# Mourtz/raytracer-0

Measured on AMD Instinct MI355X. Metric: Msamples/sec (pixels x spp / s) at 1024^2 Cornell, 8 bounces, higher is better.
Workload: dtype f32; 1 GPU; c2 (c2_cornell_mis_8): BASELINE configs[1] (the headline): 1024x1024 Cornell, MIS power heuristic, MAX_BOUNCES = MAX_DIFF_BOUNCES = 8, 64 spp; width=1024, height=1024, spp=64, max_diff_bounces=8, parallelism=row-band x1 (16-row bands), kernel=scene-specialised (hipRTC JIT), executor_compat=False

## Files before the change

raytracer-0_amd/csrc/rt0_integrator.h:

```cpp
#pragma once
#ifndef RT0_JIT
#include <hip/hip_runtime.h>
#include "rt0_device.h"
#endif

#define DEV __device__ __forceinline__

namespace rt0 {

constexpr float EPSILON = 0.001f;
constexpr float INF_T = 1e4f;
constexpr float F_INF = __builtin_huge_valf();
constexpr float PI_F = 3.14159265f;
constexpr float ONE_OVER_PI = 0.31830989f;
constexpr float TWO_PI = 6.28318531f;
constexpr float FOUR_PI = 12.5663706f;
constexpr float VOL_SIGMA_T = 0.15f;
constexpr float VOL_SIGMA_S = 0.13f;
constexpr float VOL_G = 0.5f;

enum { T_SPHERE = 0, T_PLANE = 1, T_BOX = 2, T_SDF = 3, T_TRIANGLE = 5 };
enum { M_LIGHT = 0, M_DIR_LIGHT = 1, M_DIFF = 2, M_SPEC = 3, M_REFR_FRESNEL = 4, M_REFR_SCHLICK = 5, M_COAT = 6 };

struct v3 {
  float x, y, z;
};
DEV v3 mk(float x, float y, float z) { return v3{x, y, z}; }
DEV v3 operator+(v3 a, v3 b) { return mk(a.x + b.x, a.y + b.y, a.z + b.z); }
DEV v3 operator-(v3 a, v3 b) { return mk(a.x - b.x, a.y - b.y, a.z - b.z); }
DEV v3 operator*(v3 a, v3 b) { return mk(a.x * b.x, a.y * b.y, a.z * b.z); }
DEV v3 operator*(v3 a, float s) { return mk(a.x * s, a.y * s, a.z * s); }
DEV float dot(v3 a, v3 b) { return a.x * b.x + a.y * b.y + a.z * b.z; }
DEV float frcp(float x) { return __builtin_amdgcn_rcpf(x); }
DEV float frsq(float x) { return __builtin_amdgcn_rsqf(x); }
DEV float fsqrt(float x) { return __builtin_amdgcn_sqrtf(x); }
DEV float fdiv(float a, float b) { return a * frcp(b); }
DEV float sgn(float x) { return x > 0.0f ? 1.0f : (x < 0.0f ? -1.0f : 0.0f); }
DEV float step_(float e, float x) { return x < e ? 0.0f : 1.0f; }
DEV float mixf(float x, float y, float a) { return a * (y - x) + x; }
DEV v3 normalize(v3 a) { return a * frsq(dot(a, a)); }
DEV float length(v3 a) { return fsqrt(dot(a, a)); }
DEV v3 vmaxs(v3 a, float s) { return mk(fmaxf(a.x, s), fmaxf(a.y, s), fmaxf(a.z, s)); }
DEV float vmaxc(v3 a) { return fmaxf(a.x, fmaxf(a.y, a.z)); }
DEV v3 vabs(v3 a) { return mk(fabsf(a.x), fabsf(a.y), fabsf(a.z)); }
DEV v3 reflect(v3 i, v3 n) { return i - n * (2.0f * dot(n, i)); }
DEV v3 refract(v3 i, v3 n, float eta) {
  float d = dot(n, i);
  float k = 1.0f - eta * eta * (1.0f - d * d);
  if (k < 0.0f) return mk(0.f, 0.f, 0.f);
  return i * eta - n * (eta * d + fsqrt(k));
}
DEV float fsin(float x) { return __sinf(x); }
DEV float fcos(float x) { return __cosf(x); }
DEV float fsin_rev(float t) { return __builtin_amdgcn_sinf(t); }
DEV float fcos_rev(float t) { return __builtin_amdgcn_cosf(t); }
DEV float fexp(float x) { return __expf(x); }
DEV float flog(float x) { return __logf(x); }

#ifndef RT0_HALO_CHECK
#define RT0_HALO_CHECK 1
#endif
#ifndef RT0_DEFER_NEE
#define RT0_DEFER_NEE 0
#endif
#ifndef RT0_NEE_REGIONS
#define RT0_NEE_REGIONS 2
#endif
#ifndef RT0_TAP_BATCH
#define RT0_TAP_BATCH 1
#endif
#ifndef RT0_NEE_WALK
#define RT0_NEE_WALK 0
#endif
#ifndef RT0_WALK_ROOT_TEST
#define RT0_WALK_ROOT_TEST 1
#endif
#define RT0_RES_STRIDE 2
#ifndef RT0_TREELET
#define RT0_TREELET 0
#endif
#ifndef RT0_BVH_STACK16
#define RT0_BVH_STACK16 0
#endif
#ifndef RT0_WAVEFRONT
#define RT0_WAVEFRONT 0
#endif
#ifndef RT0_WF_REFILL
#define RT0_WF_REFILL 1
#endif
#ifndef RT0_WF_WALK_REFILL
#define RT0_WF_WALK_REFILL 16
#endif
#ifndef RT0_WF_INLINE_NODES
#define RT0_WF_INLINE_NODES 1
#endif
#ifndef RT0_WF_UNIT
#define RT0_WF_UNIT 256
#endif
DEV float nc_fract(float x) {
#pragma clang fp contract(off)
  return x - floorf(x);
}
DEV float nc_addmul(float a, float b, float c) {
#pragma clang fp contract(off)
  return a + (b * c);
}
DEV float nc_seed4(float s, float a, float f, float b, float c, float d) {
#pragma clang fp contract(off)
  return ((s + (a * f)) + b) + (c * d);
}
DEV float nc_seed3(float s, float a, float f, float c, float d) {
#pragma clang fp contract(off)
  return (s + (a * f)) + (c * d);
}

DEV float hash(float seed) {
#pragma clang fp contract(off)
  uint32_t n = __float_as_uint(seed) * 747796405u + 2891336453u;
  n = ((n >> ((n >> 28u) + 4u)) ^ n) * 277803737u;
  const uint32_t m = (n >> 22u) ^ n;
  const float lo = (float)(int32_t)(m & 0x7fffffffu);
  const float hi = __int_as_float((int32_t)m >> 31 & 0x3f000000);
  return __builtin_fmaf(lo, 2.3283064365386963e-10f, hi);
}
DEV void hash2(float sx, float sy, float &ox, float &oy) {
#pragma clang fp contract(off)
  float x = (sx * 0.1031f), y = (sy * 0.1030f);
  x = x - floorf(x);
  y = y - floorf(y);
  float d = (x * (y + 19.19f)) + (y * (x + 19.19f));
  x += d;
  y += d;
  float a = ((x + y) * x), b = ((x + y) * y);
  ox = a - floorf(a);
  oy = b - floorf(b);
}

struct DynScene {
  static constexpr bool kStatic = false;
  static constexpr int kMeshes = 0, kSdfs = 0, kLights = 0;
  static constexpr bool kMayHaveModels = true;
  const SceneDev *__restrict__ S;
  DEV int n_meshes() const { return S->n_meshes; }
  DEV int n_sdfs() const { return S->n_sdfs; }
  DEV int n_models() const { return S->n_models; }
  DEV int n_lights() const { return S->n_lights; }
  DEV GeomRec geom(int i) const { return S->geom[i]; }
  DEV MatRec mat(int i) const { return S->mat[i]; }
  DEV float j3(int i) const { return S->j3[i]; }
  DEV int sdf_kind(int i) const { return S->sdf_kind[i]; }
  DEV int light(int i) const { return S->light_index[i]; }
  DEV bool any_tex() const { return S->any_tex != 0; }
  DEV TexRec tex(int i) const { return S->tex[i]; }
};

struct DynCfg {
  uint32_t fl;
  int mb, md, ms, mt, msc, mst, rs;
  float fud;
  DEV explicit DynCfg(const LaunchParams &P)
      : fl(P.flags), mb(P.max_bounces), md(P.max_diff), ms(P.max_spec), mt(P.max_trans), msc(P.max_scatter),
        mst(P.marching_steps), rs(P.restir_samples), fud(P.fudge) {}
  DEV uint32_t flags() const { return fl; }
  DEV int max_bounces() const { return mb; }
  DEV int max_diff() const { return md; }
  DEV int max_spec() const { return ms; }
  DEV int max_trans() const { return mt; }
  DEV int max_scatter() const { return msc; }
  DEV int marching_steps() const { return mst; }
  DEV int restir_samples() const { return rs; }
  DEV float fudge() const { return fud; }
};

template <int I, int N, class F>
DEV void static_for(F &&f) {
  if constexpr (I < N) {
    f(I);
    static_for<I + 1, N>(f);
  }
}
template <class Scene, class F>
DEV void for_meshes(const Scene &sc, F &&f) {
  if constexpr (Scene::kStatic) static_for<0, Scene::kMeshes>(f);
  else
    for (int i = 0; i < sc.n_meshes(); ++i) f(i);
}
template <class Scene, class F>
DEV void for_lights(const Scene &sc, F &&f) {
  if constexpr (Scene::kStatic) static_for<0, Scene::kLights>(f);
  else
    for (int i = 0; i < sc.n_lights(); ++i) f(i);
}
template <class Scene, class F>
DEV void for_sdfs(const Scene &sc, F &&f) {
  if constexpr (Scene::kStatic) static_for<0, Scene::kSdfs>(f);
  else
    for (int i = 0; i < sc.n_sdfs(); ++i) f(i);
}

struct Hit {
  v3 n, pos;
  int index;
  int type;
};

#ifndef RT0_MARCH_BUDGET
#define RT0_MARCH_BUDGET 12
#endif

struct March {
  v3 o, d;
  float tmin, t, id;
  int i;
  bool active, done;
  v3 n;
};

DEV v3 ray_at(v3 o, v3 d, float t) {
  return v3{__builtin_fmaf(d.x, t, o.x), __builtin_fmaf(d.y, t, o.y), __builtin_fmaf(d.z, t, o.z)};
}

DEV float sdBox(v3 p, v3 b) {
  v3 d = vabs(p) - b;
  v3 m = mk(fmaxf(d.x, 0.f), fmaxf(d.y, 0.f), fmaxf(d.z, 0.f));
  return length(m) + fminf(fmaxf(d.x, fmaxf(d.y, d.z)), 0.0f);
}
DEV float sdCone(v3 p, v3 c) {
  float qx = fsqrt(p.x * p.x + p.z * p.z), qy = p.y;
  float d1 = -qy - c.z;
  float d2 = fmaxf(qx * c.x + qy * c.y, qy);
  float a = fmaxf(d1, 0.f), b = fmaxf(d2, 0.f);
  return fsqrt(a * a + b * b) + fminf(fmaxf(d1, d2), 0.f);
}
DEV float gmod(float x, float y) { return x - y * floorf(x * frcp(y)); }
DEV float menger(v3 p, v3 scale) {
  float d = sdBox(p, scale);
  float s = 1.0f;
#pragma unroll
  for (int m = 0; m < 4; ++m) {
    v3 ps = p * s;
    v3 a = mk(gmod(ps.x, 2.0f) - 1.0f, gmod(ps.y, 2.0f) - 1.0f, gmod(ps.z, 2.0f) - 1.0f);
    s *= 3.0f;
    v3 r = mk(fabsf(1.0f - 3.0f * fabsf(a.x)), fabsf(1.0f - 3.0f * fabsf(a.y)), fabsf(1.0f - 3.0f * fabsf(a.z)));
    float da = fmaxf(r.x, r.y), db = fmaxf(r.y, r.z), dc = fmaxf(r.z, r.x);
    float c = (fminf(da, fminf(db, dc)) - 1.0f) / s;
    d = fmaxf(c, d);
  }
  return d;
}
DEV float mandelbulb(v3 p) {
// ... 1648 lines not shown
      spec = true;
    } else if (mt.type == M_COAT) {
      float nt_eff = fabsf(mt.nt);
      if constexpr (SPECTRAL) {
        if (flag(F_SPECTRAL) && mt.nt < 0.0f) nt_eff = spectral_ior(hero, fabsf(mt.nt));
      }
      spec = hash(seed) < schlick(gr_rd, gr_nl, 1.00029f, nt_eff);
    }
    if (spec || !flag(F_SAMPLE_LIGHTS) || !flag(F_RESTIR_DEF)) return;
    if (flag(F_RESTIR) && flag(F_MIS)) {
      if (sc.n_lights() <= 8) return;
    } else if (!flag(F_RESTIR)) {
      return;
    }
    const float fr = (float)frame;
    restir<true>(gr_x, gr_nl, mt, nc_seed3(seed, 8652.1f, fr, gr_bounce, 7895.13f),
                 nc_seed3(seed, 1234.567f, fr, gr_bounce, 9876.54f));
  }
  DEV bool ghost_on() const { return RESTIR && (C.flags() & F_EXEC_GHOST) != 0; }

  DEV bool quad_rec() const { return !RESTIR && (C.flags() & F_EXEC_GHOST) != 0 && P.quad_mode != 0; }
  DEV int light_q(int i, float bounce) {
    const int li = sc.light(i);
    if (!quad_rec()) return li;
    const int d = (int)bounce;
    if (d >= 32) return li;
    if (i == 0) q_own |= 1u << d;
    if (!q0_on || sc.n_lights() < 2) return li;
    const uint32_t m = q0_m | (flag(F_VOL) ? 0u : q0_g);
    if ((m >> d) & 1u) return li;
    if (flag(F_VOL) && (m & ((1u << d) - 1u)) == 0u) return sc.light(0);
    return 0;
  }
  DEV void quad_ghost(float seed, int depth) {
    if (!gr_have || depth >= 32) return;
    const MatRec mt = sc.mat(gr_mat);
    bool spec = gr_spec;
    if (mt.type == M_DIFF) {
      spec = false;
    } else if (mt.type == M_SPEC || mt.type == M_REFR_FRESNEL || mt.type == M_REFR_SCHLICK) {
      spec = true;
    } else if (mt.type == M_COAT) {
      float nt_eff = fabsf(mt.nt);
      if constexpr (SPECTRAL) {
        if (flag(F_SPECTRAL) && mt.nt < 0.0f) nt_eff = spectral_ior(hero, fabsf(mt.nt));
      }
      spec = hash(seed) < schlick(gr_rd, gr_nl, 1.00029f, nt_eff);
    }
    if (!spec && flag(F_SAMPLE_LIGHTS) && !flag(F_RESTIR) && !(flag(F_MIS) && sc.n_lights() > 0) &&
        sc.n_lights() <= 4)
      q_gown |= 1u << depth;
  }
  DEV void quad_begin() {
    if (!quad_rec()) return;
    q_own = q_gown = 0u;
    gr_have = false;
    q0_on = P.quad_mode == 2 && ((q_px | q_py) & 1) != 0;
    if (q0_on) {
      const uint2 m = P.quad_masks[(size_t)(q_py & ~1) * P.width + (q_px & ~1)];
      q0_m = m.x;
      q0_g = m.y;
    }
  }
  DEV void quad_store() const {
    if (quad_rec() && P.quad_mode == 1) P.quad_masks[(size_t)q_py * P.width + q_px] = make_uint2(q_own, q_gown);
  }

  DEV void wf_emit_shadow(int l, v3 o, v3 d, float tq, v3 c, bool dirl) {
    const uint32_t i = wave_append(wf_wave_counter(1));
    float4 *e = P.wf_sh + 3 * ((size_t)wf_region * (uint32_t)P.wf_R * (uint32_t)P.wf_L + i);
    e[0] = make_float4(o.x, o.y, o.z, tq);
    e[1] = make_float4(d.x, d.y, d.z, __uint_as_float((uint32_t)l * P.wf_slots + wf_slot));
    e[2] = make_float4(c.x, c.y, c.z, dirl ? 1.0f : 0.0f);
    wf_bits |= 1u << l;
  }
  DEV void wf_nee_surface(v3 x, v3 nl, float seed, float bounce) {
    if (flag(F_RESTIR)) return;
    const float fr = (float)frame;
    const float base = nc_seed4(seed, 8652.1f, fr, 5681.123f, bounce, 7895.13f);
    wf_kind = 1;
    for_lights(sc, [&](int i) {
      const int idx = sc.light(i);
      if (idx < 0) return;
      WfShadow wj{mk(0.f, 0.f, 0.f), mk(0.f, 0.f, 0.f), -1.0f, false};
      if (flag(F_MIS)) {
        const GeomRec lg = sc.geom(idx);
        const MatRec lmt = sc.mat(idx);
        if (lmt.type != M_LIGHT) return;
        LightGeo geo{false, 0.f, 0.f, 0.f, mk(0.f, 0.f, 0.f)};
        const v3 ls = direct_light(idx, x, nl, nc_addmul(base, (float)i, 123.456f), nullptr, nullptr, &geo, false, &wj);
        if (!(dot(ls, ls) > 0.000001f) || wj.tq < 0.0f) return;
        float w;
        if (geo.sphere && !flag(F_ANIM)) {
          float lp = 0.0f;
          if (geo.d2 > geo.r2 && 1.0f - geo.cam >= 1e-6f) lp = frcp(TWO_PI * (1.0f - geo.cam));
          w = power_heuristic(lp, cos_pdf(geo.ld, nl));
        } else {
          const v3 ld = normalize(lpos(idx, lg) - x);
          w = power_heuristic(light_pdf(lg, lmt, x), cos_pdf(ld, nl));
        }
        wf_emit_shadow(i, wj.o, wj.d, wj.tq, ls * w, wj.dirl);
      } else {
        const v3 dl = direct_light(idx, x, nl, base, nullptr, nullptr, nullptr, false, &wj);
        if ((dl.x != 0.0f || dl.y != 0.0f || dl.z != 0.0f) && wj.tq >= 0.0f) wf_emit_shadow(i, wj.o, wj.d, wj.tq, dl, wj.dirl);
      }
    });
  }
  DEV void wf_nee_volume(v3 sp, v3 rd, v3 mask, float seed, int depth) {
    wf_kind = 2;
    for_lights(sc, [&](int li) {
      const int lidx = sc.light(li);
      if (lidx < 0) return;
      const GeomRec lg = sc.geom(lidx);
      const MatRec lmt = sc.mat(lidx);
      if (lmt.type != M_LIGHT || lg.type != T_SPHERE) return;
      v3 dlc = mk(lg.px, lg.py, lg.pz) - sp;
      float dc = length(dlc);
      float cam = fsqrt(1.0f - fminf(fmaxf(fdiv(lg.d0, dc * dc), 0.0f), 1.0f));
      float idc = frcp(dc);
      v3 dir = sample_cone(mk(dlc.x * idc, dlc.y * idc, dlc.z * idc), 1.0f - cam,
                           nc_addmul(nc_addmul(seed + 2341.7f, (float)li, 917.3f), (float)depth, 199.1f));
      Hit sh;
      const v3 so = sp + dir * (EPSILON * 20.0f);
      float ts = isect_q(so, dir, sh);
      if (sh.index != lidx) return;
      float omega = 2.0f * (1.0f - cam);
      float ct = dot(rd, dir);
      constexpr float g2 = VOL_G * VOL_G;
      float den = 1.0f + g2 - 2.0f * VOL_G * ct;
      float phase = fdiv(1.0f - g2, FOUR_PI * den * fsqrt(den));
      float Tf = fexp(-VOL_SIGMA_T * ts);
      const v3 c = ((((mask * mk(lmt.cr, lmt.cg, lmt.cb)) * mk(lmt.er, lmt.eg, lmt.eb)) * phase) * Tf) * (PI_F * omega);
      wf_emit_shadow(li, so, dir, ts, c, false);
    });
  }

  static constexpr bool WF = RT0_WAVEFRONT != 0 && SDF && !RESTIR && !COUNT;
  static constexpr bool SUSP = SDF && !RESTIR && !COUNT && !WF;
  static constexpr bool WFB = RT0_WAVEFRONT != 0 && RESTIR && !SDF && !COUNT && Scene::kMayHaveModels;
  struct NeeCtx {
    v3 x, n, acc;
    float seed;
    int li;
    bool vol, end;
  };
  struct Path {
    v3 ro, rd, acc, mask, prev_nl;
    float seed;
    int depth;
    bool spec;
    int phase;
    March ms;
    NeeCtx nc;
  };
  DEV March *march_slot(Path &ps) {
    if constexpr (WFB) return (sc.n_models() > 0 && P.n_tris > 0) ? &ps.ms : nullptr;
    if constexpr (!SUSP && !WF) return nullptr;
    if constexpr (Scene::kMayHaveModels)
      if (sc.n_models() > 0 && P.n_tris > 0) return nullptr;
    return &ps.ms;
  }
  DEV void march_pending(Path &ps) {
    March &m = ps.ms;
    if (!m.active) return;
    const int cap = C.marching_steps();
    float t = m.t, id = m.id;
    int i = m.i;
    const int lim = min(cap, i + RT0_MARCH_BUDGET);
    bool stop = i >= cap;
    for (; i < lim; ++i) {
      float dist = G::map(sc, ray_at(m.o, m.d, t), id, n_map);
      float h = fabsf(dist);
      if (h < EPSILON || t > m.tmin) {
        stop = true;
        break;
      }
      t = __builtin_fmaf(h, C.fudge(), t);
    }
    if (i >= cap) stop = true;
    m.t = t;
    m.id = id;
    m.i = i;
    if (stop) {
      m.active = false;
      m.done = true;
    }
  }
  DEV bool nee_phase(Path &ps) {
    NeeCtx &nc = ps.nc;
    March *mq = march_slot(ps);
    bool susp = false;
    if (VOL && nc.vol) {
      const v3 sp = nc.x, rd = nc.n;
      const float seed = ps.seed;
      const int depth = ps.depth;
      for_lights(sc, [&](int li) {
        if (susp || li < nc.li) return;
        int lidx = sc.light(li);
        if (lidx < 0) return;
        const GeomRec lg = sc.geom(lidx);
        const MatRec lmt = sc.mat(lidx);
        if (lmt.type != M_LIGHT || lg.type != T_SPHERE) return;
        v3 dlc = mk(lg.px, lg.py, lg.pz) - sp;
        float dc = length(dlc);
        float cam = fsqrt(1.0f - fminf(fmaxf(fdiv(lg.d0, dc * dc), 0.0f), 1.0f));
        float idc = frcp(dc);
        v3 dir = sample_cone(mk(dlc.x * idc, dlc.y * idc, dlc.z * idc), 1.0f - cam,
                             nc_addmul(nc_addmul(seed + 2341.7f, (float)li, 917.3f), (float)depth, 199.1f));
        Hit sh;
        float ts = isect(sp + dir * (EPSILON * 20.0f), dir, sh, mq);
        if (mq && ts < 0.0f) {
          nc.li = li;
          susp = true;
          return;
        }
        if (sh.index != lidx) return;
        float omega = 2.0f * (1.0f - cam);
        float ct = dot(rd, dir);
        constexpr float g2 = VOL_G * VOL_G;
        float den = 1.0f + g2 - 2.0f * VOL_G * ct;
        float phase = fdiv(1.0f - g2, FOUR_PI * den * fsqrt(den));
        float Tf = fexp(-VOL_SIGMA_T * ts);
        ps.acc = ps.acc + ((((ps.mask * mk(lmt.cr, lmt.cg, lmt.cb)) * mk(lmt.er, lmt.eg, lmt.eb)) * phase) * Tf) *
                              (PI_F * omega);
      });
      return !susp;
    }
    if (!flag(F_RESTIR)) {
      if (flag(F_MIS) && sc.n_lights() > 0) {
        for_lights(sc, [&](int i) {
          if (susp || i < nc.li) return;
          int idx = light_q(i, (float)ps.depth);
          if (idx < 0) return;
          const GeomRec lg = sc.geom(idx);
          const MatRec lmt = sc.mat(idx);
          if (lmt.type != M_LIGHT) return;
          v3 ls = direct_light(idx, nc.x, nc.n, nc_addmul(nc.seed, (float)i, 123.456f), mq, &susp);
          if (susp) {
            nc.li = i;
            return;
          }
          if (dot(ls, ls) > 0.000001f) {
            v3 ld = normalize(lpos(idx, lg) - nc.x);
            nc.acc = nc.acc + ls * power_heuristic(light_pdf(lg, lmt, nc.x), cos_pdf(ld, nc.n));
          }
        });
      } else {
        for_lights(sc, [&](int i) {
          if (susp || i < nc.li) return;
          int idx = light_q(i, (float)ps.depth);
          if (idx < 0) return;
          v3 dl = direct_light(idx, nc.x, nc.n, nc.seed, mq, &susp);
          if (susp) {
            nc.li = i;
            return;
          }
          nc.acc = nc.acc + dl;
        });
      }
    }
    if (susp) return false;
    ps.acc = ps.acc + nc.acc * ps.mask;
    return true;
  }
  DEV bool step(Path &ps) {
    if constexpr (SUSP) {
      if (ps.phase == 1) {
        if (!nee_phase(ps)) return true;
        ps.phase = 0;
        return ps.nc.end ? false : ++ps.depth < C.max_bounces();
      }
    }
    v3 &ro = ps.ro, &rd = ps.rd, &acc = ps.acc, &mask = ps.mask, &prev_nl = ps.prev_nl;
    bool &spec = ps.spec;
    const float seed = ps.seed;
    const int depth = ps.depth;
    const float fr = (float)frame;
    {
    if (COUNT) ++n_iter;
    Hit hit;
    float t = isect(ro, rd, hit, march_slot(ps));
    if ((SUSP || WF || WFB) && t < 0.0f) return true;
    if constexpr (VOL) {
      if (flag(F_VOL)) {
        float sd = -flog(fmaxf(hash(nc_addmul(seed + 4729.3f, (float)depth, 991.1f)), 1e-6f)) / VOL_SIGMA_T;
        if (sd < fminf(INF_T, t)) {
          v3 sp = ro + rd * sd;
          mask = mask * (VOL_SIGMA_S / VOL_SIGMA_T);
          if constexpr (WF) {
            const v3 rd_in = rd;
            rd = sample_hg(rd, nc_addmul(seed + 8293.7f, (float)depth, 773.3f));
            ro = sp;
            spec = false;
            ++scat_ev;
            const bool stop = scat_ev >= C.max_scatter() || vmaxc(mask) < 0.01f;
            if (flag(F_SAMPLE_LIGHTS)) wf_nee_volume(sp, rd_in, mask, seed, depth);
            return stop ? false : ++ps.depth < C.max_bounces();
          }
          if constexpr (SUSP) {
            const v3 rd_in = rd;
            rd = sample_hg(rd, nc_addmul(seed + 8293.7f, (float)depth, 773.3f));
            ro = sp;
            spec = false;
            ++scat_ev;
            const bool stop = scat_ev >= C.max_scatter() || vmaxc(mask) < 0.01f;
            if (flag(F_SAMPLE_LIGHTS)) {
              ps.nc = NeeCtx{sp, rd_in, mk(0.f, 0.f, 0.f), seed, 0, true, stop};
              ps.phase = 1;
              if (!nee_phase(ps)) return true;
              ps.phase = 0;
            }
            return stop ? false : ++ps.depth < C.max_bounces();
          }
          if (flag(F_SAMPLE_LIGHTS)) {
            for_lights(sc, [&](int li) {
              int lidx = sc.light(li);
              if (lidx < 0) return;
              const GeomRec lg = sc.geom(lidx);
              const MatRec lmt = sc.mat(lidx);
              if (lmt.type != M_LIGHT || lg.type != T_SPHERE) return;
              v3 dlc = mk(lg.px, lg.py, lg.pz) - sp;
              float dc = length(dlc);
              float cam = fsqrt(1.0f - fminf(fmaxf(fdiv(lg.d0, dc * dc), 0.0f), 1.0f));
              float idc = frcp(dc);
              v3 dir = sample_cone(mk(dlc.x * idc, dlc.y * idc, dlc.z * idc), 1.0f - cam,
                                   nc_addmul(nc_addmul(seed + 2341.7f, (float)li, 917.3f), (float)depth, 199.1f));
              if (COUNT) ++n_nee;
              Hit sh;
              float ts = isect(sp + dir * (EPSILON * 20.0f), dir, sh);
              if (sh.index != lidx) return;
              float omega = 2.0f * (1.0f - cam);
              float ct = dot(rd, dir);
              constexpr float g2 = VOL_G * VOL_G;
              float den = 1.0f + g2 - 2.0f * VOL_G * ct;
              float phase = fdiv(1.0f - g2, FOUR_PI * den * fsqrt(den));
              float Tf = fexp(-VOL_SIGMA_T * ts);
              acc = acc + ((((mask * mk(lmt.cr, lmt.cg, lmt.cb)) * mk(lmt.er, lmt.eg, lmt.eb)) * phase) * Tf) *
                              (PI_F * omega);
            });
          }
          rd = sample_hg(rd, nc_addmul(seed + 8293.7f, (float)depth, 773.3f));
          ro = sp;
          spec = false;
          ++scat_ev;
          if (scat_ev >= C.max_scatter() || vmaxc(mask) < 0.01f) {
            if (ghost_on()) ghost_brdf(seed);
            else if (quad_rec()) quad_ghost(seed, depth);
            return false;
          }
          return ++ps.depth < C.max_bounces();
        }
      }
    }
    if (t == INF_T) {
      if (ghost_on()) ghost_brdf(seed);
      else if (quad_rec()) quad_ghost(seed, depth);
      if (!spec && flag(F_SAMPLE_LIGHTS)) return false;
      if (flag(F_CUBEMAP)) {
        const T4 cm = cube_sample(P, rd);
        acc = acc + mask * mk(cm.r, cm.g, cm.b);
      } else if (flag(F_SKY)) {
        float k = fminf(fmaxf(rd.y * 0.6f + 0.5f, 0.3f), 1.0f);
        v3 sky = mk(0.5f + 0.5f * fcos(TWO_PI * (0.525f + 0.9f * k)), 0.5f + 0.5f * fcos(TWO_PI * (0.408f + 0.97f * k)),
                    0.5f + 0.5f * fcos(TWO_PI * (0.409f + 0.8f * k)));
        acc = acc + mask * sky;
      }
      return false;
    }
    const GeomRec g = geom_at(hit.index);
    const MatRec mt = mat_at(hit.index);
    v3 c = mk(mt.cr, mt.cg, mt.cb), e = mk(mt.er, mt.eg, mt.eb);
    bool pre = false;
    if constexpr (Scene::kStatic) {
      if constexpr (!Scene::any_tex()) {
        const MatRec ms = mat_shade_at(hit.index);
        c = mk(ms.cr, ms.cg, ms.cb);
        e = mk(ms.er, ms.eg, ms.eb);
        pre = true;
      }
    }
    if (sc.any_tex()) {
      const TexRec tr = sc.tex(hit.index);
      if (tr.type >= 0 && (tr.opts & 3u)) {
        const T4 tx = hit_texel(P, tr, hit);
        if (tr.opts & 1u) {
          const float a = tx.a;
          c = mk(mixf(c.x, tx.r * tr.cmr, a), mixf(c.y, tx.g * tr.cmg, a), mixf(c.z, tx.b * tr.cmb, a));
        }
        if (tr.opts & 2u) {
          const float a = tx.a;
          e = mk(mixf(e.x, tx.r * tr.emr, a), mixf(e.y, tx.g * tr.emg, a), mixf(e.z, tx.b * tr.emb, a));
        }
      }
    }
    if (!pre) c = vmaxs(c, 0.001f);
    float inside = -sgn(dot(rd, hit.n));
    if (!pre) e = vmaxs(e, 0.001f);
    if (mt.type == M_LIGHT) {
      mask = mask * c;
      float w = 1.0f;
      if (flag(F_MIS) && !spec && flag(F_SAMPLE_LIGHTS) && depth > 0) {
        v3 ld = normalize(hit.pos - ro);
        w = power_heuristic(cos_pdf(ld, prev_nl), light_pdf(g, mt, ro));
      }
      acc = acc + (mask * e) * w;
      if (ghost_on()) ghost_brdf(seed);
      else if (quad_rec()) quad_ghost(seed, depth);
      return false;
    }
    prev_nl = hit.n * inside;

    const v3 x = hit.pos;
    const v3 nl = hit.n * inside;
    const float bounce = (float)depth;
    v3 rdir;
    {
      float s = nc_seed4(seed, 7.1f, fr, 5681.123f, bounce, 92.13f);
      rdir = flag(F_BIASED) ? sample_cosine(nl, s) : sample_cone(nl, 1.0f, s);
    }
    const float ncr = 1.00029f;
    float nt_eff = fabsf(mt.nt);
    if constexpr (SPECTRAL) {
      if (flag(F_SPECTRAL) && mt.nt < 0.0f) nt_eff = spectral_ior(hero, fabsf(mt.nt));
    }
    const int mtype = mt.type;
    if (mtype == M_DIFF) {
      ro = x + nl * EPSILON;
      rd = rdir;
      mask = mask * c;
      ++diff_b;
      spec = false;
    } else if (mtype == M_SPEC) {
      ro = x + nl * EPSILON;
      rd = normalize(e * rdir + reflect(rd, nl));
      mask = mask * c;
      ++spec_b;
      spec = true;
    } else if (mtype == M_REFR_FRESNEL || mtype == M_REFR_SCHLICK) {
      float nnt = inside < 0.0f ? fdiv(nt_eff, ncr) : fdiv(ncr, nt_eff);
      v3 tdir = refract(rd, nl, nnt);
      if (dot(tdir, tdir) == 0.0f) {
        ro = x + nl * EPSILON;
        rd = normalize(e * rdir + reflect(rd, nl));
        ++spec_b;
        spec = true;
      } else {
        tdir = normalize(e * rdir + tdir);
        float Re = mtype == M_REFR_FRESNEL ? fresnel(rd, nl, ncr, nt_eff, tdir) : schlick(rd, nl, ncr, nt_eff);
        if (hash(seed) < Re) {
          ro = x + nl * EPSILON;
          rd = normalize(e * rdir + reflect(rd, nl));
          ++spec_b;
        } else {
          ro = x - nl * EPSILON;
          mask = mask * c;
          rd = tdir;
          ++scat_ev;
        }
        spec = true;
      }
    } else if (mtype == M_COAT) {
      ro = x + nl * EPSILON;
      if (hash(seed) < schlick(rd, nl, ncr, nt_eff)) {
        rd = normalize(e * rdir + reflect(rd, nl));
        ++spec_b;
        spec = true;
      } else {
        rd = rdir;
        mask = mask * c;
        ++diff_b;
        spec = false;
      }
    }
    if (quad_rec()) {
      gr_have = true;
      gr_nl = nl;
      gr_rd = rd;
      gr_spec = spec;
      gr_mat = hit.index;
    }
    if (!spec && flag(F_CUBEMAP)) {
      const float s = nc_addmul(seed, bounce, 965.325f);
      const v3 sr = flag(F_BIASED) ? sample_cosine(nl, s) : sample_cone(nl, 1.0f, s);
      Hit eh;
      if (isect(x + nl * EPSILON, sr, eh) == INF_T) {
        const T4 cm = cube_sample(P, sr);
        acc = acc + mask * mk(cm.r, cm.g, cm.b);
      }
    }
    if constexpr (WF) {
      const bool end = vmaxc(mask) < 0.01f || diff_b >= C.max_diff() || spec_b >= C.max_spec() || 0 >= C.max_trans() ||
                       scat_ev >= C.max_scatter();
      if (!spec && flag(F_SAMPLE_LIGHTS)) wf_nee_surface(x, nl, seed, bounce);
      return end ? false : ++ps.depth < C.max_bounces();
    }
    if constexpr (SUSP) {
      const bool end = vmaxc(mask) < 0.01f || diff_b >= C.max_diff() || spec_b >= C.max_spec() || 0 >= C.max_trans() ||
                       scat_ev >= C.max_scatter();
      if (!spec && flag(F_SAMPLE_LIGHTS)) {
        ps.nc = NeeCtx{x, nl, mk(0.f, 0.f, 0.f), nc_seed4(seed, 8652.1f, fr, 5681.123f, bounce, 7895.13f), 0, false, end};
        ps.phase = 1;
        if (!nee_phase(ps)) return true;
        ps.phase = 0;
      }
      return end ? false : ++ps.depth < C.max_bounces();
    }
    if (!spec && flag(F_SAMPLE_LIGHTS)) {
      if constexpr (RT0_DEFER_NEE && RESTIR && !COUNT) {
        if (restir_routed()) defer_nee(x, nl, hit.index, seed, bounce, mask);
        else acc = acc + sample_lights(x, nl, mt, seed, bounce) * mask;
      } else {
        acc = acc + sample_lights(x, nl, mt, seed, bounce) * mask;
      }
    }
    if (ghost_on()) {
      gr_have = true;
      gr_x = x;
      gr_nl = nl;
      gr_rd = rd;
      gr_spec = spec;
      gr_bounce = bounce;
      gr_mat = hit.index;
    }

    if (vmaxc(mask) < 0.01f) return false;
    if (diff_b >= C.max_diff() || spec_b >= C.max_spec() || 0 >= C.max_trans() || scat_ev >= C.max_scatter()) return false;
    }
    return ++ps.depth < C.max_bounces();
  }

  DEV v3 radiance(v3 ro, v3 rd, float seed) {
    Path ps{ro, rd, mk(0.f, 0.f, 0.f), mk(1.f, 1.f, 1.f), mk(0.f, 1.f, 0.f), seed, 0, true};
    if (C.max_bounces() > 0)
      while (step(ps)) {
        if constexpr (SUSP) march_pending(ps);
      }
    return ps.acc;
  }

  DEV float pixel_seed() const {
#pragma clang fp contract(off)
    return hash(((fcx * 12.9898f) + (fcy * 78.233f)) + (1113.1f * (float)frame));
  }
  DEV void restir_seeds(int bounce, float &sx, float &sy) const {
    const float seed = pixel_seed(), fr = (float)frame, b = (float)bounce;
    sx = nc_seed3(seed, 8652.1f, fr, b, 7895.13f);
    sy = nc_seed3(seed, 1234.567f, fr, b, 9876.54f);
  }
  DEV void set_pixel(int px, int py) {
    q_px = px;
    q_py = py;
    fcx = (float)px + 0.5f;
    fcy = (float)py + 0.5f;
    stx = 2.0f * fcx / P.res_x - 1.0f;
    sty = 2.0f * fcy / P.res_y - 1.0f;
  }
  DEV void begin(Path &ps, int px, int py) {
    set_pixel(px, py);
    begin_sample(ps);
  }
  DEV void begin_sample(Path &ps) {
    diff_b = spec_b = scat_ev = 0;
    const float seed = pixel_seed();
    hero = 550.0f;
    if constexpr (SPECTRAL) {
      if (flag(F_SPECTRAL)) hero = nc_addmul(380.0f, hash(seed + 4821.73f), 340.0f);
    }
    const v3 u = mk(P.ux, P.uy, P.uz), v = mk(P.vx, P.vy, P.vz), w = mk(P.wx, P.wy, P.wz);
    const float ax = hash(seed + 13.271f), ay = hash(seed + 63.216f);
    const float flx = step_(0.5f, ax), fly = step_(0.5f, ay);
    const float hx = mixf(ax, 1.0f - ax, flx), hy = mixf(ay, 1.0f - ay, fly);
    const float sx = fsqrt(2.0f * hx), sy = fsqrt(2.0f * hy);
    const float dx = mixf(sx - 1.0f, 1.0f - sx, flx) * (1.0f / (P.res_x * 0.5f)) + stx;
    const float dy = mixf(sy - 1.0f, 1.0f - sy, fly) * (1.0f / (P.res_y * 0.5f)) + sty;
    const v3 fp = normalize(((u * dx) * P.uULen + (v * dy) * P.uVLen) + w) * P.focal;
    v3 ro = mk(P.cam_px, P.cam_py, P.cam_pz), rd;
    if (P.aperture != 0.0f) {
      const float ang = hash(seed + 496.4562f);
      const float rad = hash(seed + 249.1686f) * P.aperture;
      const v3 ap = (u * fcos_rev(ang) + v * fsin_rev(ang)) * rad;
      ro = ro + ap;
      rd = normalize(fp - ap);
    } else {
      rd = normalize(fp);
    }
    if (RESTIR) {
      fin = empty_res();
      gr_have = false;
      nee_k = 0;
    }
    quad_begin();
    ps = Path{ro, rd, mk(0.f, 0.f, 0.f), mk(1.f, 1.f, 1.f), mk(0.f, 1.f, 0.f), seed, 0, true};
  }
  DEV v3 finish(const Path &ps) {
    v3 col = ps.acc;
    if constexpr (SPECTRAL) {
      if (flag(F_SPECTRAL)) col = col * wavelength_to_rgb(hero);
    }
    return col;
  }
  DEV v3 sample(int px, int py) {
    Path ps;
    begin(ps, px, py);
    if (C.max_bounces() > 0)
      while (step(ps)) {
        if constexpr (SUSP) march_pending(ps);
      }
    return finish(ps);
  }
};

DEV int image_row(const LaunchParams &P, int r) {
  const int b = r / P.band;
  return (b * P.n_shards + P.shard) * P.band + (r - b * P.band);
}

template <class It>
DEV void accumulate(const It &it, const LaunchParams &P, float4 &a, v3 s) {
  if (it.flag(F_ANIM)) {
    a.x = mixf(a.x, s.x, P.ema_alpha);
    a.y = mixf(a.y, s.y, P.ema_alpha);
    a.z = mixf(a.z, s.z, P.ema_alpha);
  } else {
#pragma clang fp contract(off)
    a.x += (s.x);
    a.y += (s.y);
    a.z += (s.z);
  }
}

DEV size_t sample_plane(const LaunchParams &P) { return (size_t)(P.vp_x1 - P.vp_x0) * (P.vp_y1 - P.vp_y0); }
DEV size_t sample_index(const LaunchParams &P, int px, int r) {
  return (size_t)(r - P.vp_y0) * (P.vp_x1 - P.vp_x0) + (px - P.vp_x0);
}


template <class It, class Cfg>
DEV void regen_pixel(const LaunchParams &P, It &it, const Cfg &cfg, int px, int py, size_t apix) {
  float4 a = P.accum[apix];
  if (P.nframes > 0) {
    typename It::Path ps;
    int f = 0;
    it.frame = P.frame0;
    it.begin(ps, px, py);
    bool alive = cfg.max_bounces() > 0;
    while (true) {
      if (alive && !(It::SUSP && ps.ms.active)) alive = it.step(ps);
      if (!alive) {
        accumulate(it, P, a, it.finish(ps));
        it.quad_store();
        if (++f >= P.nframes) break;
        it.frame = P.frame0 + (uint32_t)f;
        it.begin_sample(ps);
        alive = cfg.max_bounces() > 0;
      }
      if constexpr (It::SUSP) it.march_pending(ps);
    }
  }
  P.accum[apix] = a;
}

template <class Scene, class Cfg, bool RESTIR, bool VOL, bool SDF, bool SPECTRAL, bool COUNT>
DEV void pass_body(const LaunchParams &P, Scene sc, Cfg cfg) {
  treelet_load(P);
  static_assert(!Integrator<Scene, Cfg, RESTIR, VOL, SDF, SPECTRAL, COUNT>::WF &&
                    !Integrator<Scene, Cfg, RESTIR, VOL, SDF, SPECTRAL, COUNT>::WFB,
                "RT0_WAVEFRONT modules render through wf_shade_body / wf_restir_shade_body");
  const SceneTables tabs = scene_tables(sc);
  const int lane = threadIdx.x & 63, wave = threadIdx.x >> 6;
  const int lx = (lane & 7) + ((wave & 1) << 3);
  const int ly = (lane >> 3) + ((wave >> 1) << 3);
  const int px = P.vp_x0 + (int)blockIdx.x * 16 + lx;
  const int r = P.vp_y0 + (int)blockIdx.y * 16 + ly;
  if (px >= P.vp_x1 || r >= P.vp_y1) return;
  const int py = image_row(P, r);
  if (py >= P.height) return;
  Integrator<Scene, Cfg, RESTIR, VOL, SDF, SPECTRAL, COUNT> it(P, sc, cfg);
  it.use_tables(tabs);
  const size_t pix = (size_t)py * P.width + px;
  const size_t apix = P.compact ? (size_t)r * P.width + px : pix;
  if (!RESTIR && P.samples) {
    const int f0 = (int)blockIdx.z * P.frame_chunk;
    const int f1 = min(P.nframes, f0 + P.frame_chunk);
    const size_t plane = sample_plane(P), lp = sample_index(P, px, r);
    for (int f = f0; f < f1; ++f) {
      it.frame = P.frame0 + (uint32_t)f;
      v3 s = it.sample(px, py);
      P.samples[(size_t)f * plane + lp] = make_float4(s.x, s.y, s.z, 0.f);
    }
  } else if constexpr (!RESTIR && !COUNT) {
    regen_pixel(P, it, cfg, px, py, apix);
  } else if constexpr (RT0_DEFER_NEE && RESTIR && !COUNT) {
    it.frame = P.frame0;
    it.nee_pix = (int32_t)pix;
    it.nee_wave = (blockIdx.y * gridDim.x + blockIdx.x) * 4u + (uint32_t)wave;
    volatile uint32_t *wc = nee_wave_counter();
    *wc = 0u;
    typename decltype(it)::Path ps;
    it.begin(ps, px, py);
    if (cfg.max_bounces() > 0)
      while (it.step(ps)) {
      }
    const uint32_t total = *wc;
    if (lane == __ffsll((long long)__ballot(1)) - 1) P.nee_count[it.nee_wave] = total;
    P.nee_partial[pix] = make_float4(ps.acc.x, ps.acc.y, ps.acc.z, it.hero);
    P.nee_n[pix] = it.nee_k;
    if (it.nee_k > 0) return;
  } else {
    float4 a = P.accum[apix];
    for (int f = 0; f < P.nframes; ++f) {
      it.frame = P.frame0 + (uint32_t)f;
      accumulate(it, P, a, it.sample(px, py));
    }
    P.accum[apix] = a;
  }
  if constexpr (RESTIR) {
    if (P.rout_main == nullptr || P.rout_aux == nullptr) return;
    if (it.flag(F_RESTIR_DEF)) {
      const Res &q = it.fin;
      P.rout_main[RT0_RES_STRIDE * (size_t)pix] = make_float4(q.pos.x, q.pos.y, q.pos.z, q.W);
      P.rout_aux[RT0_RES_STRIDE * (size_t)pix] = make_float4(q.col.x, q.col.y, q.col.z, pack_alpha(q.age, q.M, q.idx, sc.n_lights()));
    } else {
      P.rout_main[RT0_RES_STRIDE * (size_t)pix] = make_float4(0.f, 0.f, 0.f, 0.f);
      P.rout_aux[RT0_RES_STRIDE * (size_t)pix] = make_float4(0.f, 0.f, 0.f, 0.f);
    }
  }
  if constexpr (COUNT) {
    atomicAdd(&P.counters[0], it.n_isect);
    atomicAdd(&P.counters[1], it.n_iter);
    atomicAdd(&P.counters[2], it.n_nee);
    atomicAdd(&P.counters[3], it.n_map);
    atomicAdd(&P.counters[4], (unsigned long long)P.nframes);
    atomicAdd(&P.counters[5], it.n_restir);
    atomicAdd(&P.counters[6], it.n_cand);
    atomicAdd(&P.counters[7], it.n_ttap);
    atomicAdd(&P.counters[8], it.n_stap);
    atomicAdd(&P.counters[9], it.n_bvh[0]);
    atomicAdd(&P.counters[10], it.n_bvh[1]);
  }
}

template <class Scene, class Cfg>
DEV const float4 *candidate_table(const Scene &sc, const Cfg &cfg) {
  if constexpr (Scene::kStatic && Scene::kLights > 0) {
    if constexpr ((Cfg::flags() & F_ANIM) == 0u) {
      __shared__ float4 cand[2 * Scene::kLights];
      for (int k = (int)threadIdx.x; k < Scene::kLights; k += (int)blockDim.x) {
        const int li = sc.light(k);
        const bool ok = li >= 0 && li < sc.n_meshes() + sc.n_sdfs();
        const GeomRec lg = sc.geom(ok ? li : 0);
        const MatRec lmt = sc.mat(ok ? li : 0);
        const v3 lc = mk(lmt.cr, lmt.cg, lmt.cb) * mk(lmt.er, lmt.eg, lmt.eb);
        cand[2 * k] = make_float4(lg.px, lg.py, lg.pz, lc.x);
        cand[2 * k + 1] = make_float4(lc.y, lc.z, __int_as_float(ok ? li : -1), 0.f);
      }
      __syncthreads();
      return cand;
    }
  }
  (void)sc;
  (void)cfg;
  return nullptr;
}

#ifndef RT0_FUSED_RESOLVE
#define RT0_FUSED_RESOLVE 0
#endif
template <class Cfg, bool SPECTRAL>
DEV void resolve_pixel(const LaunchParams &P, const Cfg &cfg, int px, int r);

template <class Scene, class Cfg, bool VOL, bool SDF, bool SPECTRAL>
DEV void nee_body(const LaunchParams &P, Scene sc, Cfg cfg) {
  treelet_load(P);
  const float4 *cand = candidate_table(sc, cfg);
  const SceneTables tabs = scene_tables(sc);
  const uint32_t r0 = (uint32_t)__builtin_amdgcn_readfirstlane((int)(blockIdx.x * 4u + (threadIdx.x >> 6))) *
                      RT0_NEE_REGIONS;
  if (r0 >= (uint32_t)P.nee_regions) return;
  uint32_t cnt[RT0_NEE_REGIONS], total = 0;
#pragma unroll
  for (int q = 0; q < RT0_NEE_REGIONS; ++q) {
    cnt[q] = r0 + q < (uint32_t)P.nee_regions ? min(P.nee_count[r0 + q], (uint32_t)P.nee_cap) : 0u;
    total += cnt[q];
  }
  const size_t plane = (size_t)P.width * P.height;
  using It = Integrator<Scene, Cfg, true, VOL, SDF, SPECTRAL, false>;
  auto slot_of = [&](uint32_t i) -> size_t {
    uint32_t q = 0, off = i;
#pragma unroll
    for (int k = 0; k < RT0_NEE_REGIONS - 1; ++k)
      if (q == (uint32_t)k && off >= cnt[k]) {
        off -= cnt[k];
        q = k + 1;
      }
    return (size_t)(r0 + q) * (uint32_t)P.nee_cap + off;
  };
  auto setup = [&](It &it, const NeeRec &r) {
    it.cand_lds = cand;
    it.use_tables(tabs);
    it.frame = P.frame0;
    const int py = r.pix / P.width, px = r.pix - py * P.width;
    it.fcx = (float)px + 0.5f;
    it.fcy = (float)py + 0.5f;
    it.fin = empty_res();
    it.gr_have = false;
  };
  auto store = [&](const NeeRec &r, v3 c, const Res &q) {
    P.nee_out[(size_t)r.k() * plane + r.pix] = make_float4(c.x * r.mr, c.y * r.mg, c.z * r.mb, 0.f);
    if (r.k() == P.nee_n[r.pix] - 1 && P.rout_main != nullptr && P.rout_aux != nullptr) {
      P.rout_main[RT0_RES_STRIDE * (size_t)r.pix] = make_float4(q.pos.x, q.pos.y, q.pos.z, q.W);
      P.rout_aux[RT0_RES_STRIDE * (size_t)r.pix] = make_float4(q.col.x, q.col.y, q.col.z, pack_alpha(q.age, q.M, q.idx, sc.n_lights()));
    }
  };
#if RT0_NEE_WALK
  WalkJob *wj = P.walk_jobs + (size_t)(r0 / RT0_NEE_REGIONS) * (2u * RT0_NEE_REGIONS * (uint32_t)P.nee_cap);
  uint32_t njob = 0;
  const uint32_t lane = threadIdx.x & 63u;
  const uint64_t lt = (1ull << lane) - 1ull;
  for (uint32_t base = 0; base < total; base += 64u) {
    const uint32_t i = base + lane;
    bool has0 = false, has1 = false;
    WalkJob j0, j1;
    if (i < total) {
      const size_t slot = slot_of(i);
      const NeeRec r = P.nee_rec[slot];
      It it(P, sc, cfg);
      setup(it, r);
      float sx, sy;
      it.restir_seeds(r.bounce(), sx, sy);
      const auto sp = it.restir_split(mk(r.x, r.y, r.z), mk(r.nx, r.ny, r.nz), it.mat_at(r.mat()), sx, sy);
      if (sp.done) {
        store(r, sp.c, it.fin);
      } else {
        bool w0 = sp.has[0], w1 = sp.has[1];
        if constexpr (RT0_WALK_ROOT_TEST) {
          auto miss = [&](const WalkJob &j) {
            return bvh_root_miss(P, mk(j.ox, j.oy, j.oz), mk(frcp(j.dx), frcp(j.dy), frcp(j.dz)), j.tmax);
          };
          w0 = w0 && !miss(sp.j[0]);
          w1 = w1 && !miss(sp.j[1]);
        }
        const int tag = (w0 || w1) ? (int)(((uint32_t)slot + 1u) << 2) | (w0 ? 1 : 0) | (w1 ? 2 : 0) : 0;
        P.nee_out[(size_t)r.k() * plane + r.pix] =
            make_float4(sp.f.x * r.mr, sp.f.y * r.mg, sp.f.z * r.mb, __int_as_float(tag));
// ... 723 lines not shown
```

Before: 13220 Msamples/s.

## Defer light-hit emission to path end and use per-frame sample loop

When a path hits a light, it now records the light index and hit distance and exits the bounce loop. The emission and MIS weight are then computed once, after the loop, in a new path_end routine. This keeps the light-hit branch out of the divergent inner loop. The regenerating per-lane sample loop is also replaced by a plain per-frame outer loop, which trades lane-level refill for simpler control flow but can leave lanes idle until the slowest path in a wave finishes.

```diff
diff --git a/raytracer-0_amd/csrc/rt0_integrator.h b/raytracer-0_amd/csrc/rt0_integrator.h
--- a/raytracer-0_amd/csrc/rt0_integrator.h
+++ b/raytracer-0_amd/csrc/rt0_integrator.h
@@ -96,6 +96,9 @@
 #endif
 #ifndef RT0_WF_UNIT
 #define RT0_WF_UNIT 256
+#endif
+#ifndef RT0_PATH_END_DEFER
+#define RT0_PATH_END_DEFER 1
 #endif
 DEV float nc_fract(float x) {
 #pragma clang fp contract(off)
@@ -2050,7 +2053,61 @@
     int phase;
     March ms;
     NeeCtx nc;
+    int end_mesh;
+    float end_t;
   };
+  DEV bool defer_end() const {
+    if constexpr (!RT0_PATH_END_DEFER || RESTIR || COUNT || SUSP || WF || WFB) return false;
+    else return !ghost_on() && !quad_rec() && !sc.any_tex();
+  }
+  DEV void path_end(Path &ps) {
+    if (!defer_end() || ps.end_mesh == 0) return;
+    const int idx = ps.end_mesh - 1;
+    const GeomRec g = geom_at(idx);
+    const MatRec mt = mat_at(idx);
+    v3 c, e;
+    if constexpr (Scene::kStatic) {
+      const MatRec ms = mat_shade_at(idx);
+      c = mk(ms.cr, ms.cg, ms.cb);
+      e = mk(ms.er, ms.eg, ms.eb);
+    } else {
+      c = vmaxs(mk(mt.cr, mt.cg, mt.cb), 0.001f);
+      e = vmaxs(mk(mt.er, mt.eg, mt.eb), 0.001f);
+    }
+    const v3 me = (ps.mask * c) * e;
+    float w = 1.0f;
+    if (flag(F_MIS) && !ps.spec && flag(F_SAMPLE_LIGHTS) && ps.depth > 0) w = light_hit_weight(ps, g, mt);
+    ps.acc = mk(__builtin_fmaf(me.x, w, ps.acc.x), __builtin_fmaf(me.y, w, ps.acc.y), __builtin_fmaf(me.z, w, ps.acc.z));
+  }
+  DEV float dot_yxz(v3 a, v3 b) const {
+#pragma clang fp contract(off)
+    return __builtin_fmaf(a.z, b.z, __builtin_fmaf(a.x, b.x, a.y * b.y));
+  }
+  DEV float light_hit_weight(const Path &ps, const GeomRec &g, const MatRec &mt) const {
+#pragma clang fp contract(off)
+    const v3 ro = ps.ro;
+    const v3 pos = mk(__builtin_fmaf(ps.rd.x, ps.end_t, ro.x), __builtin_fmaf(ps.rd.y, ps.end_t, ro.y),
+                      __builtin_fmaf(ps.rd.z, ps.end_t, ro.z));
+    const v3 d = mk(pos.x - ro.x, pos.y - ro.y, pos.z - ro.z);
+    const float r = frsq(dot_yxz(d, d));
+    const v3 ld = mk(d.x * r, d.y * r, d.z * r);
+    const float f = fmaxf(0.0f, dot_yxz(ld, ps.prev_nl)) * ONE_OVER_PI;
+    float lp = 0.0f;
+    if (mt.type == M_LIGHT) {
+      if (g.type == T_SPHERE) {
+        const v3 dc = mk(g.px - ro.x, g.py - ro.y, g.pz - ro.z);
+        const float d2 = dot_yxz(dc, dc), r2 = g.d0;
+        if (!(d2 <= r2)) {
+          const float den = 1.0f - fsqrt(fmaxf(0.0f, __builtin_fmaf(-r2, frcp(d2), 1.0f)));
+          if (!(den < 1e-6f)) lp = frcp(TWO_PI * den);
+        }
+      } else {
+        lp = 1.0f / FOUR_PI;
+      }
+    }
+    const float ff = f * f;
+    return fmaxf(0.0f, ff * frcp(__builtin_fmaf(lp, lp, ff)));
+  }
   DEV March *march_slot(Path &ps) {
     if constexpr (WFB) return (sc.n_models() > 0 && P.n_tris > 0) ? &ps.ms : nullptr;
     if constexpr (!SUSP && !WF) return nullptr;
@@ -2295,6 +2352,11 @@
     float inside = -sgn(dot(rd, hit.n));
     if (!pre) e = vmaxs(e, 0.001f);
     if (mt.type == M_LIGHT) {
+      if (defer_end()) {
+        ps.end_mesh = hit.index + 1;
+        ps.end_t = t;
+        return false;
+      }
       mask = mask * c;
       float w = 1.0f;
       if (flag(F_MIS) && !spec && flag(F_SAMPLE_LIGHTS) && depth > 0) {
@@ -2433,6 +2495,7 @@
       while (step(ps)) {
         if constexpr (SUSP) march_pending(ps);
       }
+    path_end(ps);
     return ps.acc;
   }
 
@@ -2504,6 +2567,7 @@
       while (step(ps)) {
         if constexpr (SUSP) march_pending(ps);
       }
+    path_end(ps);
     return finish(ps);
   }
 };
@@ -2534,26 +2598,24 @@
 
 
 template <class It, class Cfg>
-DEV void regen_pixel(const LaunchParams &P, It &it, const Cfg &cfg, int px, int py, size_t apix) {
+DEV void pixel_passes(const LaunchParams &P, It &it, const Cfg &cfg, int px, int py, size_t apix) {
   float4 a = P.accum[apix];
-  if (P.nframes > 0) {
-    typename It::Path ps;
-    int f = 0;
-    it.frame = P.frame0;
-    it.begin(ps, px, py);
-    bool alive = cfg.max_bounces() > 0;
-    while (true) {
-      if (alive && !(It::SUSP && ps.ms.active)) alive = it.step(ps);
-      if (!alive) {
-        accumulate(it, P, a, it.finish(ps));
-        it.quad_store();
-        if (++f >= P.nframes) break;
-        it.frame = P.frame0 + (uint32_t)f;
-        it.begin_sample(ps);
-        alive = cfg.max_bounces() > 0;
-      }
-      if constexpr (It::SUSP) it.march_pending(ps);
-    }
+  typename It::Path ps;
+  it.set_pixel(px, py);
+  for (int f = 0; f < P.nframes; ++f) {
+    it.frame = P.frame0 + (uint32_t)f;
+    it.begin_sample(ps);
+    if (cfg.max_bounces() > 0) {
+      if constexpr (It::SUSP) {
+        while (ps.ms.active || it.step(ps)) it.march_pending(ps);
+      } else {
+        while (it.step(ps)) {
+        }
+      }
+    }
+    it.path_end(ps);
+    accumulate(it, P, a, it.finish(ps));
+    it.quad_store();
   }
   P.accum[apix] = a;
 }
@@ -2587,7 +2649,7 @@
       P.samples[(size_t)f * plane + lp] = make_float4(s.x, s.y, s.z, 0.f);
     }
   } else if constexpr (!RESTIR && !COUNT) {
-    regen_pixel(P, it, cfg, px, py, apix);
+    pixel_passes(P, it, cfg, px, py, apix);
   } else if constexpr (RT0_DEFER_NEE && RESTIR && !COUNT) {
     it.frame = P.frame0;
     it.nee_pix = (int32_t)pix;
```

Result: faster. 13500 Msamples/s (median of 6 runs) (+2.2%).
